# phymhan/pc-gan

Measured on AMD Instinct MI355X. Metric: images/sec (G+D step) 128x128 bs32 per GPU, higher is better.
Workload: dtype f32; 1 GPU; wsgan_emb UTKFace-shaped 128x128 bs32/GPU fp32: 9-block ResnetGenerator + 3-layer PatchGAN + ResNet-18 Elo encoder@224 + AlexNet IP@224, full optimize_parameters(); global_batch=32, parallelism=dp1

## Files before the change

### include/pcgan_hip.h

```cpp
#ifndef PCGAN_HIP_H
#define PCGAN_HIP_H

#include <stddef.h>
#include <stdint.h>

#ifdef __cplusplus
extern "C" {
#endif

typedef void* pcgan_stream_t;

const char* pcgan_last_error(void);
int pcgan_version(void);
int pcgan_device_info(int* cu_count, char* arch, int arch_len);

typedef struct {
    int N, C, H, W;
    int K, R, S;
    int stride, pad, pad_mode;
    int P, Q;
    int dtype;
} pcgan_conv_desc;

enum { PCGAN_ACT_NONE = 0, PCGAN_ACT_RELU = 1, PCGAN_ACT_LRELU = 2, PCGAN_ACT_TANH = 3, PCGAN_ACT_SIGMOID = 4 };
// ... 270 lines not shown
unsigned long long pcgan_pool_exchange_launches(void);

int pcgan_set_nonfinite_counter(unsigned int* dev_word);
int pcgan_set_option(const char* key, int value);
int pcgan_get_option(const char* key, int* value);
int pcgan_timer_enable(int capacity);
int pcgan_timer_read(int kind, float* ms, int cap);
#define PCGAN_IGEMM_LAUNCH_INFO 7
#define PCGAN_IGEMM_HGEMM_F16X2 1
#define PCGAN_IGEMM_HGEMM_BF16 2
#define PCGAN_IGEMM_IGEMM2_CG16 3
#define PCGAN_IGEMM_IGEMM2_CG4 4
#define PCGAN_IGEMM_GENERIC 5
#define PCGAN_IGEMM_SMALLM 6
int pcgan_igemm_last_launch(int* info, int n);
#define PCGAN_WGRAD_LAUNCH_INFO 9
#define PCGAN_WGRAD_TILE2 1
#define PCGAN_WGRAD_TILE 2
#define PCGAN_WGRAD_SMALLM 3
#define PCGAN_WGRAD_STRIP 4
int pcgan_wgrad_last_launch(int* info, int n);
#define PCGAN_HWGRAD_LAUNCH_INFO 12
int pcgan_hwgrad_last_launch(int* info, int n);

#ifdef __cplusplus
}
#endif
#endif
```

### pc-gan_amd/csrc/capi.hip

```cpp
#include "common.h"
#include <stdarg.h>
#include <atomic>
#include <mutex>
#include <vector>

namespace pcgan {
static thread_local char g_err[512] = "";
void set_error(const char* fmt, ...) {
    va_list ap;
    va_start(ap, fmt);
    vsnprintf(g_err, sizeof(g_err), fmt, ap);
    va_end(ap);
}
}

namespace pcgan {
namespace {
struct TimerKind {
    std::vector<hipEvent_t> start, stop;
    int used = 0;
};
std::mutex g_timer_mu;
std::atomic<int> g_timer_on{0};
TimerKind g_timer[TIMER_KINDS];
// ... 57 lines not shown
    }
    t.used = 0;
    return n;
}

namespace pcgan {
static std::atomic<unsigned*> g_nonfinite{nullptr};
unsigned* nonfinite_counter() { return g_nonfinite.load(std::memory_order_relaxed); }
}
extern "C" int pcgan_set_nonfinite_counter(unsigned int* dev_word) {
    pcgan::g_nonfinite.store(dev_word);
    return 0;
}

namespace pcgan {
static const char* const g_opt_names[OPT_COUNT] = {"bsplit_halo", "wgrad_gen", "wgrad_padcopy", "wgrad_cw", "hgemm_bf16", "wgd_look", "wgrad_direct", "hgemm_tile", "hgemm_ks", "wgrad_rowring", "wgrad_ks", "hwgrad_ks"};
static std::atomic<int> g_opt[OPT_COUNT] = {{1}, {1}, {0}, {0}, {1}, {3}, {0}, {0}, {0}, {1}, {0}, {0}};
int option(int id) { return (id >= 0 && id < OPT_COUNT) ? g_opt[id].load(std::memory_order_relaxed) : 0; }
static int option_index(const char* key) {
    for (int i = 0; key && i < OPT_COUNT; ++i)
        if (strcmp(key, g_opt_names[i]) == 0) return i;
    return -1;
}
}
extern "C" int pcgan_set_option(const char* key, int value) {
    using namespace pcgan;
    const int i = option_index(key);
    PCGAN_CHECK(i >= 0, "set_option: unknown option '%s' (bsplit_halo, wgrad_gen, wgrad_padcopy, wgrad_cw, hgemm_bf16, wgd_look, wgrad_direct, hgemm_tile, hgemm_ks, wgrad_rowring, wgrad_ks, hwgrad_ks)", key ? key : "(null)");
    PCGAN_CHECK(i != OPT_WGRAD_CW || value == 0 || value == 128 || value == 256, "set_option: wgrad_cw takes 0 (default), 128 or 256, got %d", value);
    PCGAN_CHECK(i != OPT_HGEMM_TILE || value == 0 || value == 128128 || value == 128064 || value == 64128 || value == 64064,
                "set_option: hgemm_tile takes 0 (heuristic) or BM * 1000 + BP with BM, BP in {64, 128}, got %d", value);
    PCGAN_CHECK(i != OPT_HGEMM_KS || (value >= 0 && value <= 8), "set_option: hgemm_ks takes 0 (heuristic) .. 8, got %d", value);
    PCGAN_CHECK(i != OPT_WGRAD_KS || (value >= 0 && value <= 512), "set_option: wgrad_ks takes 0 (heuristic) .. 512, got %d", value);
    PCGAN_CHECK(i != OPT_HWGRAD_KS || (value >= 0 && value <= 512), "set_option: hwgrad_ks takes 0 (heuristic) .. 512, got %d", value);
    g_opt[i].store(value);
    return 0;
}
extern "C" int pcgan_get_option(const char* key, int* value) {
    using namespace pcgan;
    const int i = option_index(key);
    PCGAN_CHECK(i >= 0 && value, "get_option: unknown option or null output");
    *value = g_opt[i].load();
    return 0;
// ... 20 lines not shown
```

### pc-gan_amd/csrc/common.h

```cpp
#pragma once
#include <hip/hip_runtime.h>
#include <stdint.h>
#include <stdio.h>
#include <string.h>
#include "../../include/pcgan_hip.h"

namespace pcgan {

void set_error(const char* fmt, ...);

#define PCGAN_CHECK(cond, ...)                \
    do {                                      \
        if (!(cond)) {                        \
            pcgan::set_error(__VA_ARGS__);    \
            return 1;                         \
        }                                     \
    } while (0)

#define PCGAN_LAUNCH_CHECK()                                                      \
    do {                                                                          \
        hipError_t e__ = hipGetLastError();                                       \
        if (e__ != hipSuccess) {                                                  \
            pcgan::set_error("%s:%d launch failed: %s", __FILE__, __LINE__,       \
                             hipGetErrorString(e__));                             \
// ... 1 lines not shown
        }                                                                         \
    } while (0)

enum { TIMER_RES_FWD = 0, TIMER_RES_DGRAD = 1, TIMER_RES_WGRAD = 2, TIMER_RES_WGRAD_MAIN = 3, TIMER_KINDS = 4 };
struct TimerScope {
    int kind, slot;
    hipStream_t st;
    TimerScope(int kind, hipStream_t st);
    ~TimerScope();
};

static inline int timer_kind_res(const pcgan_conv_desc* d, int kind) {
    return (d && d->K == 256 && d->C == 256 && d->R == 3 && d->S == 3 && d->stride == 1 && d->pad_mode == 1 && d->pad == 1) ? kind : -1;
}

enum { OPT_BSPLIT_HALO = 0, OPT_WGRAD_GEN = 1, OPT_WGRAD_PADCOPY = 2, OPT_WGRAD_CW = 3, OPT_HGEMM_BF16 = 4, OPT_WGD_LOOK = 5, OPT_WGRAD_DIRECT = 6, OPT_HGEMM_TILE = 7, OPT_HGEMM_KS = 8, OPT_WGRAD_ROWRING = 9, OPT_WGRAD_KS = 10, OPT_HWGRAD_KS = 11, OPT_COUNT = 12 };
int option(int id);

unsigned* nonfinite_counter();
int launch_wgd_reduce(const float* part, float* dw, const float* scales, int splits, int K, int C, int accumulate, hipStream_t st);
__device__ __forceinline__ bool is_nonfinite(float v) { return (__float_as_uint(v) & 0x7f800000u) == 0x7f800000u; }
__device__ __forceinline__ void report_nonfinite(unsigned* counter, bool bad) {
    if (counter != nullptr && __builtin_amdgcn_ballot_w64(bad) != 0ull && (threadIdx.x & 63) == 0) atomicAdd(counter, 1u);
}

int launch_weight_row_absmax(const float* w, int K, int C, int T, int by_c, float* out, hipStream_t st);

int launch_reflect_fold(const void* padded, void* dx, int NC, int H, int W, int pad, int dtype, hipStream_t st, const float* bias = nullptr,
                        int C = 1);

static inline int ilog2_exact(int v) {
// ... 176 lines not shown
```

### pc-gan_amd/csrc/hgemm.hip

```cpp
#include "igemm.h"

namespace pcgan {

typedef _Float16 f16x8 __attribute__((ext_vector_type(8)));
typedef _Float16 f16x4 __attribute__((ext_vector_type(4)));

typedef __bf16 bf16x8v __attribute__((ext_vector_type(8)));
typedef __bf16 bf16x4v __attribute__((ext_vector_type(4)));

template <int MODE, int BM, int BP, typename TA>
__global__ void __launch_bounds__(256) hgemm_kernel(IgemmArgs a) {
    static_assert(MODE == MODE_FWD_ZERO || MODE == MODE_FWD_REFLECT || MODE == MODE_BWD, "forward and plain data gradient");
    constexpr bool HALF = sizeof(TA) == 2;
    constexpr int NP = HALF ? 1 : 2;
    constexpr unsigned ES = sizeof(TA);
    constexpr int WM = (BM == 128 || (BM == 64 && BP == 64)) ? 2 : 1;
    constexpr int WP = 4 / WM;
    constexpr int WMT = BM / WM, WPT = BP / WP;
    constexpr int MI = WMT / 32, PJ = WPT / 32;
    constexpr int KPT = BP / 16;
    constexpr int ACH = BM * 4 / 256;
    constexpr int TROWS = NTAP_FWD + 1;
    constexpr int AH = BM + 8;
    __shared__ __attribute__((aligned(16))) f16x8 As[2][NP][2 * AH];
    __shared__ __attribute__((aligned(16))) f16x8 Bs[2][NP][2 * BP];
    __shared__ unsigned offT[TROWS][BP];
    __shared__ __attribute__((aligned(16))) float biasS[BM];
    __shared__ __attribute__((aligned(16))) float iswS[BM];

    const int nMt = (a.M + BM - 1) / BM;
    const int mt = blockIdx.x % nMt;
    int pt = blockIdx.x / nMt;
    int phase = 0;
    while (phase + 1 < a.nphase && pt >= a.tstart[phase + 1]) ++phase;
    pt -= a.tstart[phase];
    const PhaseArgs& P = a.ph[phase];
    const int tid = threadIdx.x;
    const int lane = tid & 63, lo = lane & 31, hi = lane >> 5;
    const int wave = __builtin_amdgcn_readfirstlane(tid >> 6);
    const int wm = wave / WP, wp = wave % WP;
    const int Ptot = P.Ptot, Kp = P.Kp;
    const int m0 = mt * BM, p0 = pt * BP;
    const int ph_nS = P.nS;
    const int T = P.nR * ph_nS;
    const int HgWg4 = a.Hg * a.Wg * (int)ES;
    const __amdgpu_buffer_rsrc_t rX = make_rsrc(a.X, a.x_bytes);
    const __amdgpu_buffer_rsrc_t rA = make_rsrc(P.A, (unsigned)a.M * (unsigned)Kp * 4u);

    float sx = 1.f;
    const int pl = tid % BP;
    {
        const int pg = p0 + pl;
        const bool pvalid = pg < Ptot;
        int gn = 0, py = 0, px = 0;
        if (pvalid) pix_coord(a, P, pg, gn, py, px);
        const unsigned vbase = (unsigned)gn * (unsigned)a.Cg * (unsigned)(a.Hg * a.Wg);
        for (int t = tid / BP; t <= T; t += 256 / BP) {
            const int ri = t / ph_nS, sj = t - ri * ph_nS;
            const int r = P.r0 + ri * a.tstep, sxx = P.s0 + sj * a.tstep;
            const bool live = pvalid && t < T;
            const unsigned y = axis_entry<MODE>(py, py + a.pad, true, r, a.Hg, a.sl, a.pad);
            const unsigned x = axis_entry<MODE>(px, px + a.pad, true, sxx, a.Wg, a.sl, a.pad);
            offT[t][pl] = (live && y != 0xffffffffu && x != 0xffffffffu) ? (vbase + y * (unsigned)a.Wg + x) * ES : OOB;
        }
    }
    const int ksub = __builtin_amdgcn_readfirstlane(tid / BP);
// ... 7 lines not shown

    int it_tap, it_c, it_k0, it_left = nst_here;
    {
        const int cc0 = st_begin / T;
        it_tap = st_begin - cc0 * T;
        it_c = cc0 * 16;
        it_k0 = st_begin * 16;
    }
    unsigned a_base[ACH];
#pragma unroll
    for (int j = 0; j < ACH; ++j) {
        const int q = tid + 256 * j;
        const int row = q >> 2, kc = (q & 3) * 4;
        a_base[j] = (m0 + row < a.M) ? (unsigned)((m0 + row) * Kp + kc) * 4u : OOB;
    }
    struct Stage {
        u32x4 av[ACH];
        unsigned bv[KPT];
    };
    auto load = [&](Stage& r) {
        const bool live = it_left > 0;
        const unsigned vo = offT[live ? it_tap : T][pl];
        const unsigned so = (unsigned)((it_c + ksub * KPT) * HgWg4);
#pragma unroll
        for (int j = 0; j < ACH; ++j) r.av[j] = __builtin_amdgcn_raw_buffer_load_b128(rA, live ? a_base[j] : OOB, (unsigned)it_k0 * 4u, 0);
#pragma unroll
        for (int i = 0; i < KPT; ++i) {
            if constexpr (HALF) r.bv[i] = (unsigned)__builtin_amdgcn_raw_buffer_load_b16(rX, vo, so + (unsigned)(i * HgWg4), 0);
            else r.bv[i] = __builtin_amdgcn_raw_buffer_load_b32(rX, vo, so + (unsigned)(i * HgWg4), 0);
        }
        --it_left;
        const int t1 = it_tap + 1;
        const bool wr = t1 == T;
        it_tap = wr ? 0 : t1;
        it_c += wr ? 16 : 0;
        it_k0 += 16;
    };
    auto stash = [&](const Stage& r, int buf) {
        if constexpr (HALF) {
#pragma unroll
            for (int j = 0; j < ACH; ++j) {
                const int q = tid + 256 * j;
                const int row = q >> 2, kc = (q & 3) * 4;
                bf16x4v h;
// ... 10 lines not shown
            return;
        }
#pragma unroll
        for (int j = 0; j < ACH; ++j) {
            const int q = tid + 256 * j;
            const int row = q >> 2, kc = (q & 3) * 4;
            typedef unsigned u32x2 __attribute__((ext_vector_type(2)));
            u32x2 h, l;
            h[0] = r.av[j][0]; h[1] = r.av[j][1];
            l[0] = r.av[j][2]; l[1] = r.av[j][3];
            _Float16* d0 = reinterpret_cast<_Float16*>(&As[buf][0][(kc >> 3) * AH + row]) + (kc & 4);
            _Float16* d1 = reinterpret_cast<_Float16*>(&As[buf][NP - 1][(kc >> 3) * AH + row]) + (kc & 4);
            *reinterpret_cast<u32x2*>(d0) = h;
            *reinterpret_cast<u32x2*>(d1) = l;
        }
        if constexpr (KPT == 8) {
            f16x8 h, l;
#pragma unroll
            for (int e = 0; e < 8; ++e) {
                _Float16 x, y;
                split2h(__uint_as_float(r.bv[e]) * sx, x, y);
                h[e] = x;
                l[e] = y;
            }
            Bs[buf][0][ksub * BP + pl] = h;
            Bs[buf][NP - 1][ksub * BP + pl] = l;
        } else {
            f16x4 h, l;
#pragma unroll
            for (int e = 0; e < 4; ++e) {
                _Float16 x, y;
// ... 4 lines not shown
            *reinterpret_cast<f16x4*>(reinterpret_cast<_Float16*>(&Bs[buf][0][(ksub >> 1) * BP + pl]) + (ksub & 1) * 4) = h;
            *reinterpret_cast<f16x4*>(reinterpret_cast<_Float16*>(&Bs[buf][NP - 1][(ksub >> 1) * BP + pl]) + (ksub & 1) * 4) = l;
        }
    };

    f32x16 acc[MI][PJ];
#pragma unroll
    for (int i = 0; i < MI; ++i)
#pragma unroll
        for (int j = 0; j < PJ; ++j)
#pragma unroll
            for (int r = 0; r < 16; ++r) acc[i][j][r] = 0.f;
    struct Operands {
        f16x8 A[NP][MI], B[NP][PJ];
    };
    auto fetch = [&](Operands& o, int buf) {
#pragma unroll
        for (int p = 0; p < NP; ++p) {
#pragma unroll
            for (int i = 0; i < MI; ++i) o.A[p][i] = As[buf][p][hi * AH + wm * WMT + i * 32 + lo];
#pragma unroll
            for (int j = 0; j < PJ; ++j) o.B[p][j] = Bs[buf][p][hi * BP + wp * WPT + j * 32 + lo];
        }
    };
    auto mma = [&](const Operands& o) {
        if constexpr (HALF) {
#pragma unroll
            for (int i = 0; i < MI; ++i)
#pragma unroll
                for (int j = 0; j < PJ; ++j)
                    acc[i][j] = __builtin_amdgcn_mfma_f32_32x32x16_bf16(__builtin_bit_cast(bf16x8v, o.A[0][i]), __builtin_bit_cast(bf16x8v, o.B[0][j]),
                                                                         acc[i][j], 0, 0, 0);
            return;
        }
        constexpr int PA[3] = {NP - 1, 0, 0}, PB[3] = {0, NP - 1, 0};
#pragma unroll
        for (int q = 0; q < 3; ++q)
#pragma unroll
            for (int i = 0; i < MI; ++i)
#pragma unroll
                for (int j = 0; j < PJ; ++j)
                    acc[i][j] = __builtin_amdgcn_mfma_f32_32x32x16_f16(o.A[PA[q]][i], o.B[PB[q]][j], acc[i][j], 0, 0, 0);
    };
    auto interleave = [&]() {
        constexpr int NM = (HALF ? 1 : 3) * MI * PJ, NRD = NP * (MI + PJ);
#pragma unroll
        for (int q = 0; q < NM; ++q) {
            __builtin_amdgcn_sched_group_barrier(0x008, 1, 0);
            __builtin_amdgcn_sched_group_barrier(0x100, (NRD + NM - 1) / NM, 0);
            __builtin_amdgcn_sched_group_barrier(0x002, 48 / NM + 1, 0);
            __builtin_amdgcn_sched_group_barrier(0x200, 1, 0);
            __builtin_amdgcn_sched_group_barrier(0x020, (ACH + KPT + NM - 1) / NM, 0);
        }
    };

    Stage rg[2];
    if (nst_here > 0) {
        load(rg[0]);
        load(rg[1]);
    }
    if constexpr (!HALF) {
        const float m = thread_max_of_partials(a.x_amax, a.x_namax, tid, 256);
        sx = pow2_scale(block_max(m, biasS));
        if (tid < BM) iswS[tid] = m0 + tid < a.M ? 1.f / pow2_scale(a.w_amax[m0 + tid]) : 1.f;
        __syncthreads();
    }
    if (tid < BM) biasS[tid] = (a.bias != nullptr && m0 + tid < a.M) ? a.bias[m0 + tid] : 0.f;
    if (nst_here == 0) __syncthreads();
    if (nst_here > 0) {
        Operands op[2];
        stash(rg[0], 0);
        __syncthreads();
        load(rg[0]);
        fetch(op[0], 0);
        stash(rg[1], 1);
        __syncthreads();
        load(rg[1]);
        const int nst2 = (nst_here + 1) & ~1;
        for (int s = 0; s < nst2; s += 2) {
#pragma unroll
            for (int t = 0; t < 2; ++t) {
                fetch(op[t ^ 1], t ^ 1);
                mma(op[t]);
                stash(rg[t], t);
                load(rg[t]);
// ... 41 lines not shown
#pragma unroll
            for (int r = 0; r < 16; ++r) {
                const int ml = wm * WMT + i * 32 + (r & 3) + 8 * (r >> 2) + 4 * hi;
                if (m0 + ml < a.M) st1(Yp + (size_t)(m0 + ml) * YhYw, act_apply((acc[i][j][r] * isx) * (HALF ? 1.f : iswS[ml]) + biasS[ml], a.act, a.slope));
            }
    }
}

template <int MODE>
static void launch_mode(const IgemmArgs& a, int bm, int bp, dim3 grid2, hipStream_t st) {
    if (bm == 128 && bp == 128) LAUNCH_TA(a.dtype, hgemm_kernel, grid2, a, MODE, 128, 128);
    else if (bm == 128) LAUNCH_TA(a.dtype, hgemm_kernel, grid2, a, MODE, 128, 64);
    else if (bp == 128) LAUNCH_TA(a.dtype, hgemm_kernel, grid2, a, MODE, 64, 128);
    else LAUNCH_TA(a.dtype, hgemm_kernel, grid2, a, MODE, 64, 64);
}
int launch_hgemm(int mode, const IgemmArgs& a, int bm, int bp, dim3 grid2, hipStream_t st) {
    switch (mode) {
        case MODE_FWD_ZERO: launch_mode<MODE_FWD_ZERO>(a, bm, bp, grid2, st); break;
        case MODE_FWD_REFLECT: launch_mode<MODE_FWD_REFLECT>(a, bm, bp, grid2, st); break;
        case MODE_BWD: launch_mode<MODE_BWD>(a, bm, bp, grid2, st); break;
        default: PCGAN_CHECK(false, "hgemm: no kernel for mode %d", mode);
    }
    PCGAN_LAUNCH_CHECK();
    return 0;
}

}

using namespace pcgan;

__global__ void __launch_bounds__(256) hgemm_presplit_kernel(float* __restrict__ A, int M, int Kp4, const float* __restrict__ rowmax) {
// ... 21 lines not shown
```

### pc-gan_amd/csrc/igemm.h

```cpp
#pragma once
#include "common.h"
#include <type_traits>

namespace pcgan {

typedef float f32x16 __attribute__((ext_vector_type(16)));

enum { MODE_FWD_ZERO = 0, MODE_FWD_REFLECT = 1, MODE_BWD = 2, MODE_BWD_REFLECT = 3 };

typedef unsigned int u32x4 __attribute__((ext_vector_type(4)));
static constexpr unsigned OOB = 0x80000000u;

__device__ __forceinline__ __amdgpu_buffer_rsrc_t make_rsrc(const void* p, unsigned bytes) {
    return __builtin_amdgcn_make_buffer_rsrc(const_cast<void*>(p), 0, (int)bytes, 0x00020000);
}
__device__ __forceinline__ float ld_b32(__amdgpu_buffer_rsrc_t r, unsigned voff, unsigned soff) {
    return __uint_as_float(__builtin_amdgcn_raw_buffer_load_b32(r, voff, soff, 0));
}
__device__ __forceinline__ float4 ld_b128(__amdgpu_buffer_rsrc_t r, unsigned voff) {
    const u32x4 v = __builtin_amdgcn_raw_buffer_load_b128(r, voff, 0, 0);
    return make_float4(__uint_as_float(v.x), __uint_as_float(v.y), __uint_as_float(v.z), __uint_as_float(v.w));
}

template <typename TA>
// ... 99 lines not shown
    int ostep, sl, pad, tstep;
    int act;
    float slope;
    unsigned x_bytes;
    int nphase;
    int rowfold;
    int chunked;
    int ksplit;
    float* Ypart;
    int tstart[17];
    PhaseArgs ph[16];
    const float* x_amax;
    const float* w_amax;
    int x_namax, hsplit;
    unsigned* ovf;
};

struct Geom {
    int Hg, Wg, sl, pad;
};

template <int MODE>
__device__ __forceinline__ bool tap_offset(const Geom& a, int py, int px, int r, int s, int& off) {
    if (MODE == MODE_BWD || MODE == MODE_BWD_REFLECT) {
        const int ty = py + a.pad - r, tx = px + a.pad - s;
        const int oy = ty >> a.sl, ox = tx >> a.sl;
        off = oy * a.Wg + ox;
        return (ty >= 0) & (tx >= 0) & (oy < a.Hg) & (ox < a.Wg);
    } else {
        int iy = (py << a.sl) - a.pad + r;
// ... 83 lines not shown
static inline int round4(int v) { return (v + 3) & ~3; }
static inline size_t esz(const pcgan_conv_desc* d) { return d->dtype == PCGAN_BF16 ? 2 : 4; }

#define LAUNCH_TA(dt, KERNEL, GRID, ARG, ...)                                                                   \
    do {                                                                                                        \
        if ((dt) == PCGAN_BF16) hipLaunchKernelGGL((KERNEL<__VA_ARGS__, bf16>), GRID, dim3(256), 0, st, ARG);    \
        else hipLaunchKernelGGL((KERNEL<__VA_ARGS__, float>), GRID, dim3(256), 0, st, ARG);                      \
    } while (0)

void record_launch(int form, int mode, int bm, int bp, int ks, int nphase);
int launch_splitk_reduce(int dtype, hipStream_t st, const float* part, void* y, const float* bias, int ks, size_t out_elems, int M,
                         int HW, int act, float slope);

int launch_igemm_f32(int mode, const IgemmArgs& a, int bm, int bp, dim3 grid, dim3 grid2, hipStream_t st);
int launch_hgemm(int mode, const IgemmArgs& a, int bm, int bp, dim3 grid2, hipStream_t st);
int launch_hgemm_presplit(float* A, int M, int Kp4, const float* rowmax, hipStream_t st);
int launch_smallm(int mode, IgemmArgs& a, int pmax, hipStream_t st, float* part_ws, size_t part_bytes);
int launch_transpose4(const float* A, float* At, int M, int Kp, hipStream_t st);
int launch_pack_strip(const float* A, float* Ws, int M, int Cg, int Cgp, int nR, int nS, hipStream_t st);
int wgrad_splits(const pcgan_conv_desc* d, int* chunks_per_split);
int launch_wgrad(const pcgan_conv_desc* d, const WgradArgs& a, int splits, float* dw, int accumulate, hipStream_t st);

}
```

### pc-gan_amd/csrc/igemm_conv.hip

```cpp
#include "igemm.h"
#include <stdlib.h>
#include <mutex>

namespace pcgan {

template <typename TA>
__global__ void splitk_reduce_kernel(const float* __restrict__ part, TA* __restrict__ y, const float* __restrict__ bias,
                                     int ks, size_t n, int M, int HW, int act, float slope) {
    const size_t n4 = (n & 3) ? 0 : (n >> 2);
    const size_t stride = (size_t)gridDim.x * blockDim.x;
    for (size_t i = blockIdx.x * (size_t)blockDim.x + threadIdx.x; i < n4; i += stride) {
        float4 acc = reinterpret_cast<const float4*>(part)[i];
        for (int s = 1; s < ks; ++s) {
            const float4 v = reinterpret_cast<const float4*>(part + (size_t)s * n)[i];
            acc.x += v.x; acc.y += v.y; acc.z += v.z; acc.w += v.w;
        }
        float o[4] = {acc.x, acc.y, acc.z, acc.w};
#pragma unroll
        for (int u = 0; u < 4; ++u) {
            const size_t e = i * 4 + u;
            if (bias) o[u] += bias[(e / HW) % M];
            o[u] = act_apply(o[u], act, slope);
        }
        st4(y + 4 * i, make_float4(o[0], o[1], o[2], o[3]));
// ... 211 lines not shown
    if (m >= 64 && tile_blocks(M, ptot_max, nphase, m, p) < 384) p = 64;
    if (m == 128 && tile_blocks(M, ptot_max, nphase, m, p) < 384) m = 64;
    *bm = m;
    *bp = p;
}

static std::mutex g_launch_mu;
static int g_launch[PCGAN_IGEMM_LAUNCH_INFO] = {0};
void record_launch(int form, int mode, int bm, int bp, int ks, int nphase) {
    std::lock_guard<std::mutex> lk(g_launch_mu);
    const int seq = g_launch[0] + 1;
    const int v[PCGAN_IGEMM_LAUNCH_INFO] = {seq, form, mode, bm, bp, ks, nphase};
    for (int i = 0; i < PCGAN_IGEMM_LAUNCH_INFO; ++i) g_launch[i] = v[i];
}

static int launch_igemm(int mode, IgemmArgs& a, hipStream_t st, float* part_ws = nullptr, size_t part_bytes = 0) {
    int pmax = 0;
    for (int i = 0; i < a.nphase; ++i) pmax = a.ph[i].Ptot > pmax ? a.ph[i].Ptot : pmax;
    if (pmax <= 0 || a.nphase <= 0) return 0;
    if (a.M <= 4) return launch_smallm(mode, a, pmax, st, part_ws, part_bytes);
    int bm, bp, ks;
    int nst_min = 1 << 30;
    for (int i = 0; i < a.nphase; ++i) nst_min = (a.ph[i].Kp + 15) / 16 < nst_min ? (a.ph[i].Kp + 15) / 16 : nst_min;
    const size_t out_elems = (size_t)a.N * a.M * a.Yh * a.Yw;
    choose_tile(a.M, pmax, a.nphase, nst_min, part_ws != nullptr, &bm, &bp, &ks);
    if (ks > 1 && (size_t)ks * out_elems * 4 > part_bytes) ks = 1;
    a.ksplit = ks;
    a.Ypart = part_ws;
    const dim3 grid((unsigned)(((a.M + bm - 1) / bm) * ((pmax + bp - 1) / bp)), (unsigned)a.nphase, (unsigned)ks);
    a.tstart[0] = 0;
// ... 3 lines not shown
    PCGAN_CHECK(cg16 || mode != MODE_BWD_REFLECT, "igemm: fused reflect data-gradient needs K %% 16 == 0");
    if (cg4) {
        PCGAN_CHECK(a.Cgp == 4, "igemm: 4-channel stages need a 3-/4-channel tensor");
        for (int i = 0; i < a.nphase; ++i)
            PCGAN_CHECK(a.ph[i].nR * a.ph[i].nS <= NTAP_CG4, "igemm: 4-channel stages: more than %d taps", NTAP_CG4);
    }
    if (cg16) {
        PCGAN_CHECK((a.Cg % 16) == 0, "igemm: chunked K order needs a multiple of 16 channels");
        for (int i = 0; i < a.nphase; ++i)
            PCGAN_CHECK(a.ph[i].nR * a.ph[i].nS <= (mode == MODE_BWD_REFLECT ? NTAP_MIR : NTAP_FWD) && (a.ph[i].Kp % 16) == 0,
                        "igemm: chunked K order: bad phase");
    }
    const bool half = a.dtype == PCGAN_BF16 && option(OPT_HGEMM_BF16) != 0;
    if ((half || (a.hsplit && a.dtype == PCGAN_F32)) && cg16 && mode != MODE_BWD_REFLECT && bm >= 64) {
        record_launch(half ? PCGAN_IGEMM_HGEMM_BF16 : PCGAN_IGEMM_HGEMM_F16X2, mode, bm, bp, ks, a.nphase);
        if (int e = launch_hgemm(mode, a, bm, bp, grid2, st)) return e;
    } else {
        record_launch(cg16 ? PCGAN_IGEMM_IGEMM2_CG16 : (cg4 ? PCGAN_IGEMM_IGEMM2_CG4 : PCGAN_IGEMM_GENERIC), mode, bm, bp, ks, a.nphase);
        if (int e = launch_igemm_f32(mode, a, bm, bp, grid, grid2, st)) return e;
    }
    if (ks > 1 && launch_splitk_reduce(a.dtype, st, part_ws, a.Y, a.bias, ks, out_elems, a.M, a.Yh * a.Yw, a.act, a.slope)) return 2;
    return 0;
}

}

using namespace pcgan;

static size_t fwd_part_bytes(const pcgan_conv_desc* d) {
    const int ptot = d->N * d->P * d->Q;
// ... 315 lines not shown
    if (fwd) return launch_hgemm_presplit(packed, M, RS * round4(d->C) / 4, w_rowmax, st);
    BwdPlan pl;
    bwd_plan(d, pl);
    for (int i = 0; i < pl.n; ++i)
        if (int e = launch_hgemm_presplit(packed + pl.ph[i].a_off, M, pl.ph[i].nR * pl.ph[i].nS * round4(d->K) / 4, w_rowmax, st)) return e;
    return 0;
}

extern "C" int pcgan_igemm_last_launch(int* info, int n) {
    PCGAN_CHECK(info != nullptr && n > 0, "igemm_last_launch: null output");
    std::lock_guard<std::mutex> lk(g_launch_mu);
    for (int i = 0; i < n; ++i) info[i] = i < PCGAN_IGEMM_LAUNCH_INFO ? g_launch[i] : 0;
    return 0;
}

extern "C" size_t pcgan_conv2d_packed_bytes(const pcgan_conv_desc* d, int pass) {
    if (!d) return 0;
    if (pass == PCGAN_PASS_FWD) return fwd_base_bytes(d);
    if (pass == PCGAN_PASS_BWD_DATA) return bwd_base_bytes(d);
    return 0;
}
extern "C" int pcgan_conv2d_pack_weights(const pcgan_conv_desc* d, int pass, const float* w, float* packed,
                                         pcgan_stream_t s) {
    if (check_desc(d)) return 1;
    PCGAN_CHECK(w && packed, "conv2d_pack_weights: null pointer");
    if (pass == PCGAN_PASS_FWD) return pack_fwd(d, w, packed, (hipStream_t)s);
    PCGAN_CHECK(pass == PCGAN_PASS_BWD_DATA, "conv2d_pack_weights: pass %d has no packed weights", pass);
    PCGAN_CHECK(d->pad_mode == 0 || d->stride == 1, "conv2d_bwd_data: reflection padding needs stride 1");
    BwdPlan pl;
    bwd_plan(d, pl);
// ... 26 lines not shown
```

### pc-gan_amd/hip/lib.py

```python
import ctypes
import os

_HERE = os.path.dirname(os.path.abspath(__file__))
LIB_PATH = os.environ.get('PCGAN_LIB') or os.path.join(os.path.dirname(_HERE), 'lib', 'libpcgan_hip.so')

ACT_NONE, ACT_RELU, ACT_LRELU, ACT_TANH, ACT_SIGMOID = 0, 1, 2, 3, 4
PASS_FWD, PASS_BWD_DATA, PASS_BWD_WEIGHT = 0, 1, 2
F32, BF16 = 0, 1
ADD_N_MAX = 8
POOL_PLAN_MAX = 64
GCAM_TYPES = {'raw': 0, 'pw': 1, 'cw_pos': 2, 'pw_cw': 3}
POOL_PASS = -1


def pool_store(s):
    return 2 * int(s)


def pool_swap(s):
    return 2 * int(s) + 1


def pool_exchange_launches():
    return int(load().pcgan_pool_exchange_launches())
# ... 97 lines not shown
    'pcgan_event_destroy': (_i, [_vp]),
    'pcgan_resblock_supported': (_i, [_rp]),
    'pcgan_resblock_wgrad_workspace_bytes': (_sz, [_rp]),
    'pcgan_resblock_fwd': (_i, [_rp, _vp, _vp, _i, _vp, _vp, _vp, _vp, _vp, _vp, _vp, _vp, _vp, _vp, _vp, _vp, _vp, _vp, _vp]),
    'pcgan_resblock_bwd': (_i, [_rp, _vp, _vp, _vp, _i, _vp, _vp, _vp, _vp, _vp, _vp, _vp, _vp, _vp, _vp, _vp, _vp, _vp, _vp, _vp, _vp,
                                _vp, _sz, _vp, _vp, _vp]),
    'pcgan_set_nonfinite_counter': (_i, [_vp]),
    'pcgan_set_option': (_i, [ctypes.c_char_p, _i]),
    'pcgan_get_option': (_i, [ctypes.c_char_p, _vp]),
    'pcgan_timer_enable': (_i, [_i]),
    'pcgan_timer_read': (_i, [_i, _vp, _i]),
    'pcgan_igemm_last_launch': (_i, [ctypes.POINTER(_i), _i]),
    'pcgan_wgrad_last_launch': (_i, [ctypes.POINTER(_i), _i]),
    'pcgan_hwgrad_last_launch': (_i, [ctypes.POINTER(_i), _i]),
    'pcgan_conv2d_hgemm_supported': (_i, [_dp, _i]),
    'pcgan_conv2d_hgemm_pack': (_i, [_dp, _i, _vp, _vp, _vp, _vp]),
    'pcgan_conv2d_fwd_packed_hsplit': (_i, [_dp, _vp, _vp, _i, _vp, _vp, _vp, _vp, _i, _f, _vp, _sz, _vp]),
    'pcgan_conv2d_bwd_data_packed_hsplit': (_i, [_dp, _vp, _vp, _i, _vp, _vp, _vp, _vp, _vp, _sz, _vp]),
    'pcgan_conv2d_thin_supported': (_i, [_dp, _i]),
    'pcgan_conv2d_thin_packed_bytes': (_sz, [_dp, _i]),
    'pcgan_conv2d_thin_workspace_bytes': (_sz, [_dp, _i]),
    'pcgan_conv2d_thin_pack': (_i, [_dp, _i, _vp, _vp, _vp]),
    'pcgan_conv2d_fwd_thin': (_i, [_dp, _vp, _vp, _i, _vp, _vp, _vp, _i, _f, _vp]),
    'pcgan_conv2d_bwd_data_thin': (_i, [_dp, _vp, _vp, _i, _vp, _vp, _vp, _sz, _vp]),
    'pcgan_conv2d_hsplit_wgrad_supported': (_i, [_dp]),
    'pcgan_conv2d_hsplit_wgrad_inline': (_i, [_dp]),
    'pcgan_conv2d_hsplit_wgrad_workspace_bytes': (_sz, [_dp]),
    'pcgan_conv2d_bwd_weight_hsplit': (_i, [_dp, _vp, _vp, _i, _vp, _vp, _i, _vp, _i, _vp, _sz, _vp]),
    'pcgan_restrunk_fwd': (_i, [_rp, _i, _vp, _vp, _i] + [_vp] * 8 + [_vp] * 6 + [_vp]),
    'pcgan_restrunk_bwd': (_i, [_rp, _i, _vp, _vp, _vp, _i] + [_vp] * 6 + [_vp] * 6 + [_vp] * 6 + [_vp, _sz, _vp, _vp, _vp]),
# ... 48 lines not shown
    bundled = os.path.join(os.path.dirname(torch.__file__), 'lib', 'libamdhip64.so')
    if os.path.exists(bundled):
        ctypes.CDLL(bundled, mode=ctypes.RTLD_GLOBAL)
    lib = ctypes.CDLL(LIB_PATH)
    for name, (res, args) in SIGNATURES.items():
        fn = getattr(lib, name)
        fn.restype = res
        fn.argtypes = args
    _lib = lib
    _options_from_environment(lib)
    return lib


_ENV_OPTIONS = (('PCGAN_BSPLIT_HALO', 'bsplit_halo', int), ('PCGAN_WGRAD_GEN', 'wgrad_gen', int), ('PCGAN_WGRAD_PADCOPY', 'wgrad_padcopy', int),
                ('PCGAN_WGRAD_CW', 'wgrad_cw', int), ('PCGAN_HGEMM', 'hgemm_bf16', int), ('PCGAN_WGRAD_DIRECT', 'wgrad_direct', int),
                ('PCGAN_WGD_LOOK', 'wgd_look', int), ('PCGAN_WGRAD_ROWRING', 'wgrad_rowring', int))


def _options_from_environment(lib):
    for env, key, conv in _ENV_OPTIONS:
        v = os.environ.get(env)
        if v not in (None, ''):
            set_option(key, conv(v), lib)


def set_option(key, value, lib=None):
    lib = lib or load()
    if lib.pcgan_set_option(key.encode(), int(value)) != 0:
        msg = lib.pcgan_last_error()
        raise RuntimeError('pcgan_hip set_option failed: %s' % (msg.decode() if msg else '?'))

# ... 13 lines not shown
```

Before: 1233 images/sec.

## Stage shared input row-span window in LDS for fp32 hgemm conv

Adds a span variant of the split-fp16 hgemm conv kernel. It loads the padded input rows covered by a pixel tile into LDS once per channel group, split into hi/lo halves, and serves every filter tap from that window. This replaces per-tap gathered global loads of the im2col B operand. The goal is to remove repeated global reads of overlapping input pixels across the R*S taps. In exchange it uses dynamic LDS, adds window-fill synchronisation and index math, and is gated by a heuristic that is on by default for zero-pad or data-grad modes when the reuse ratio is high enough.

```diff
diff --git a/include/pcgan_hip.h b/include/pcgan_hip.h
--- a/include/pcgan_hip.h
+++ b/include/pcgan_hip.h
@@ -308,6 +308,9 @@
 #define PCGAN_IGEMM_GENERIC 5
 #define PCGAN_IGEMM_SMALLM 6
 int pcgan_igemm_last_launch(int* info, int n);
+#define PCGAN_HGEMM_SPAN_INFO 5
+int pcgan_conv2d_hgemm_span_entries(const pcgan_conv_desc* d, int pass);
+int pcgan_hgemm_span_last_launch(int* info, int n);
 #define PCGAN_WGRAD_LAUNCH_INFO 9
 #define PCGAN_WGRAD_TILE2 1
 #define PCGAN_WGRAD_TILE 2
diff --git a/pc-gan_amd/csrc/capi.hip b/pc-gan_amd/csrc/capi.hip
--- a/pc-gan_amd/csrc/capi.hip
+++ b/pc-gan_amd/csrc/capi.hip
@@ -95,8 +95,8 @@
 }
 
 namespace pcgan {
-static const char* const g_opt_names[OPT_COUNT] = {"bsplit_halo", "wgrad_gen", "wgrad_padcopy", "wgrad_cw", "hgemm_bf16", "wgd_look", "wgrad_direct", "hgemm_tile", "hgemm_ks", "wgrad_rowring", "wgrad_ks", "hwgrad_ks"};
-static std::atomic<int> g_opt[OPT_COUNT] = {{1}, {1}, {0}, {0}, {1}, {3}, {0}, {0}, {0}, {1}, {0}, {0}};
+static const char* const g_opt_names[OPT_COUNT] = {"bsplit_halo", "wgrad_gen", "wgrad_padcopy", "wgrad_cw", "hgemm_bf16", "wgd_look", "wgrad_direct", "hgemm_tile", "hgemm_ks", "wgrad_rowring", "wgrad_ks", "hwgrad_ks", "hgemm_span"};
+static std::atomic<int> g_opt[OPT_COUNT] = {{1}, {1}, {0}, {0}, {1}, {3}, {0}, {0}, {0}, {1}, {0}, {0}, {1}};
 int option(int id) { return (id >= 0 && id < OPT_COUNT) ? g_opt[id].load(std::memory_order_relaxed) : 0; }
 static int option_index(const char* key) {
     for (int i = 0; key && i < OPT_COUNT; ++i)
@@ -107,7 +107,7 @@
 extern "C" int pcgan_set_option(const char* key, int value) {
     using namespace pcgan;
     const int i = option_index(key);
-    PCGAN_CHECK(i >= 0, "set_option: unknown option '%s' (bsplit_halo, wgrad_gen, wgrad_padcopy, wgrad_cw, hgemm_bf16, wgd_look, wgrad_direct, hgemm_tile, hgemm_ks, wgrad_rowring, wgrad_ks, hwgrad_ks)", key ? key : "(null)");
+    PCGAN_CHECK(i >= 0, "set_option: unknown option '%s' (bsplit_halo, wgrad_gen, wgrad_padcopy, wgrad_cw, hgemm_bf16, wgd_look, wgrad_direct, hgemm_tile, hgemm_ks, wgrad_rowring, wgrad_ks, hwgrad_ks, hgemm_span)", key ? key : "(null)");
     PCGAN_CHECK(i != OPT_WGRAD_CW || value == 0 || value == 128 || value == 256, "set_option: wgrad_cw takes 0 (default), 128 or 256, got %d", value);
     PCGAN_CHECK(i != OPT_HGEMM_TILE || value == 0 || value == 128128 || value == 128064 || value == 64128 || value == 64064,
                 "set_option: hgemm_tile takes 0 (heuristic) or BM * 1000 + BP with BM, BP in {64, 128}, got %d", value);
diff --git a/pc-gan_amd/csrc/common.h b/pc-gan_amd/csrc/common.h
--- a/pc-gan_amd/csrc/common.h
+++ b/pc-gan_amd/csrc/common.h
@@ -39,7 +39,7 @@
     return (d && d->K == 256 && d->C == 256 && d->R == 3 && d->S == 3 && d->stride == 1 && d->pad_mode == 1 && d->pad == 1) ? kind : -1;
 }
 
-enum { OPT_BSPLIT_HALO = 0, OPT_WGRAD_GEN = 1, OPT_WGRAD_PADCOPY = 2, OPT_WGRAD_CW = 3, OPT_HGEMM_BF16 = 4, OPT_WGD_LOOK = 5, OPT_WGRAD_DIRECT = 6, OPT_HGEMM_TILE = 7, OPT_HGEMM_KS = 8, OPT_WGRAD_ROWRING = 9, OPT_WGRAD_KS = 10, OPT_HWGRAD_KS = 11, OPT_COUNT = 12 };
+enum { OPT_BSPLIT_HALO = 0, OPT_WGRAD_GEN = 1, OPT_WGRAD_PADCOPY = 2, OPT_WGRAD_CW = 3, OPT_HGEMM_BF16 = 4, OPT_WGD_LOOK = 5, OPT_WGRAD_DIRECT = 6, OPT_HGEMM_TILE = 7, OPT_HGEMM_KS = 8, OPT_WGRAD_ROWRING = 9, OPT_WGRAD_KS = 10, OPT_HWGRAD_KS = 11, OPT_HGEMM_SPAN = 12, OPT_COUNT = 13 };
 int option(int id);
 
 unsigned* nonfinite_counter();
diff --git a/pc-gan_amd/csrc/hgemm.hip b/pc-gan_amd/csrc/hgemm.hip
--- a/pc-gan_amd/csrc/hgemm.hip
+++ b/pc-gan_amd/csrc/hgemm.hip
@@ -8,9 +8,10 @@
 typedef __bf16 bf16x8v __attribute__((ext_vector_type(8)));
 typedef __bf16 bf16x4v __attribute__((ext_vector_type(4)));
 
-template <int MODE, int BM, int BP, typename TA>
+template <int MODE, int BM, int BP, typename TA, bool SPAN = false>
 __global__ void __launch_bounds__(256) hgemm_kernel(IgemmArgs a) {
     static_assert(MODE == MODE_FWD_ZERO || MODE == MODE_FWD_REFLECT || MODE == MODE_BWD, "forward and plain data gradient");
+    static_assert(!SPAN || (sizeof(TA) == 4 && MODE != MODE_FWD_REFLECT), "span form: fp32 tensors, zero padding or data gradient");
     constexpr bool HALF = sizeof(TA) == 2;
     constexpr int NP = HALF ? 1 : 2;
     constexpr unsigned ES = sizeof(TA);
@@ -25,6 +26,7 @@
     __shared__ __attribute__((aligned(16))) f16x8 As[2][NP][2 * AH];
     __shared__ __attribute__((aligned(16))) f16x8 Bs[2][NP][2 * BP];
     __shared__ unsigned offT[TROWS][BP];
+    extern __shared__ __attribute__((aligned(16))) f16x8 Win[];
     __shared__ __attribute__((aligned(16))) float biasS[BM];
     __shared__ __attribute__((aligned(16))) float iswS[BM];
 
@@ -49,7 +51,34 @@
 
     float sx = 1.f;
     const int pl = tid % BP;
-    {
+    const int EW = a.span_entries + 1, pitch = a.span_pitch;
+    unsigned* const woffS = reinterpret_cast<unsigned*>(Win + 8 * EW);
+    int Et = 0, UPS = 1, eb[PJ];
+    if constexpr (SPAN) {
+        const int Hp = a.Yh + P.nR - 1;
+        int n, py, px;
+        pix_coord(a, P, p0, n, py, px);
+        const int row0 = n * Hp + py;
+        const int plast = (p0 + BP < Ptot ? p0 + BP : Ptot) - 1;
+        pix_coord(a, P, plast, n, py, px);
+        Et = (n * Hp + py + P.nR - row0) * pitch;
+        UPS = (2 * Et + 256 * T - 1) / (256 * T);
+#pragma unroll
+        for (int j = 0; j < PJ; ++j) {
+            const int pix = p0 + wp * WPT + j * 32 + lo;
+            pix_coord(a, P, pix < Ptot ? pix : Ptot - 1, n, py, px);
+            eb[j] = (n * Hp + py - row0) * pitch + px + (MODE == MODE_BWD ? (P.nR - 1) * pitch + ph_nS - 1 : 0);
+        }
+        const int oy = MODE == MODE_BWD ? P.nR - 1 - a.pad : a.pad, ox = MODE == MODE_BWD ? ph_nS - 1 - a.pad : a.pad;
+        for (int e = tid; e < Et; e += 256) {
+            const int row = e / pitch, gr = row0 + row;
+            const int gn = gr / Hp;
+            const int iy = gr - gn * Hp - oy, ix = e - row * pitch - ox;
+            const bool ok = gn < a.N && (unsigned)iy < (unsigned)a.Hg && (unsigned)ix < (unsigned)a.Wg;
+            woffS[e] = ok ? (((unsigned)gn * (unsigned)a.Cg * (unsigned)a.Hg + (unsigned)iy) * (unsigned)a.Wg + (unsigned)ix) * ES : OOB;
+        }
+        if (tid < 8) Win[tid * EW + EW - 1] = f16x8{0, 0, 0, 0, 0, 0, 0, 0};
+    } else {
         const int pg = p0 + pl;
         const bool pvalid = pg < Ptot;
         int gn = 0, py = 0, px = 0;
@@ -87,20 +116,63 @@
         const int row = q >> 2, kc = (q & 3) * 4;
         a_base[j] = (m0 + row < a.M) ? (unsigned)((m0 + row) * Kp + kc) * 4u : OOB;
     }
+    constexpr int NBV = SPAN ? 8 : KPT;
     struct Stage {
         u32x4 av[ACH];
-        unsigned bv[KPT];
-    };
+        unsigned bv[NBV];
+        int wc, wk;
+    };
+    const int c_last = st_end > st_begin ? (st_end - 1) / T : -1;
+    auto wave_has = [&](int i) { return wave * 64 + 256 * i < 2 * Et; };
+    auto win_load = [&](unsigned (&bv)[NBV], int c, int i) {
+        const int u = tid + 256 * i, kh = u >= Et ? 1 : 0;
+        const bool ok = u < 2 * Et && c <= c_last;
+        const unsigned vo = (ok ? woffS[u - kh * Et] : OOB) + (unsigned)(kh * 8 * HgWg4);
+        const unsigned so = (unsigned)(c * 16 * HgWg4);
+#pragma unroll
+        for (int e = 0; e < 8; ++e) bv[e] = __builtin_amdgcn_raw_buffer_load_b32(rX, vo, so + (unsigned)(e * HgWg4), 0);
+    };
+    auto win_put = [&](const unsigned (&bv)[NBV], int c, int i) {
+        const int u = tid + 256 * i, kh = u >= Et ? 1 : 0;
+        if (u >= 2 * Et) return;
+        f16x8 h, l;
+#pragma unroll
+        for (int e = 0; e < 8; ++e) {
+            _Float16 x, y;
+            split2h(__uint_as_float(bv[e]) * sx, x, y);
+            h[e] = x;
+            l[e] = y;
+        }
+        f16x8* const w = Win + ((c & 1) * 4 + kh) * EW + (u - kh * Et);
+        w[0] = h;
+        w[2 * EW] = l;
+    };
+    auto win_sync = [&](int c, int i) {
+        if (!wave_has(i)) return;
+        unsigned bv[NBV];
+        win_load(bv, c, i);
+        win_put(bv, c, i);
+    };
+    int wi_c = (st_begin - 1 + T) / T, wi_k = (st_begin - 1 + T) % T;
     auto load = [&](Stage& r) {
         const bool live = it_left > 0;
-        const unsigned vo = offT[live ? it_tap : T][pl];
-        const unsigned so = (unsigned)((it_c + ksub * KPT) * HgWg4);
 #pragma unroll
         for (int j = 0; j < ACH; ++j) r.av[j] = __builtin_amdgcn_raw_buffer_load_b128(rA, live ? a_base[j] : OOB, (unsigned)it_k0 * 4u, 0);
-#pragma unroll
-        for (int i = 0; i < KPT; ++i) {
-            if constexpr (HALF) r.bv[i] = (unsigned)__builtin_amdgcn_raw_buffer_load_b16(rX, vo, so + (unsigned)(i * HgWg4), 0);
-            else r.bv[i] = __builtin_amdgcn_raw_buffer_load_b32(rX, vo, so + (unsigned)(i * HgWg4), 0);
+        if constexpr (SPAN) {
+            r.wc = wi_c;
+            r.wk = wi_k;
+            if (wave_has(wi_k * UPS)) win_load(r.bv, wi_c, wi_k * UPS);
+            const bool ww = wi_k + 1 == T;
+            wi_k = ww ? 0 : wi_k + 1;
+            wi_c += ww ? 1 : 0;
+        } else {
+            const unsigned vo = offT[live ? it_tap : T][pl];
+            const unsigned so = (unsigned)((it_c + ksub * KPT) * HgWg4);
+#pragma unroll
+            for (int i = 0; i < KPT; ++i) {
+                if constexpr (HALF) r.bv[i] = (unsigned)__builtin_amdgcn_raw_buffer_load_b16(rX, vo, so + (unsigned)(i * HgWg4), 0);
+                else r.bv[i] = __builtin_amdgcn_raw_buffer_load_b32(rX, vo, so + (unsigned)(i * HgWg4), 0);
+            }
         }
         --it_left;
         const int t1 = it_tap + 1;
@@ -141,7 +213,10 @@
             *reinterpret_cast<u32x2*>(d0) = h;
             *reinterpret_cast<u32x2*>(d1) = l;
         }
-        if constexpr (KPT == 8) {
+        if constexpr (SPAN) {
+            if (wave_has(r.wk * UPS)) win_put(r.bv, r.wc, r.wk * UPS);
+            for (int j = 1; j < UPS; ++j) win_sync(r.wc, r.wk * UPS + j);
+        } else if constexpr (KPT == 8) {
             f16x8 h, l;
 #pragma unroll
             for (int e = 0; e < 8; ++e) {
@@ -176,13 +251,32 @@
     struct Operands {
         f16x8 A[NP][MI], B[NP][PJ];
     };
+    int f_r = (st_begin % T) / ph_nS, f_s = (st_begin % T) % ph_nS, f_buf = (st_begin / T) & 1, f_left = nst_here;
+    int f_toff = f_r * pitch + f_s;
     auto fetch = [&](Operands& o, int buf) {
 #pragma unroll
         for (int p = 0; p < NP; ++p) {
 #pragma unroll
             for (int i = 0; i < MI; ++i) o.A[p][i] = As[buf][p][hi * AH + wm * WMT + i * 32 + lo];
-#pragma unroll
-            for (int j = 0; j < PJ; ++j) o.B[p][j] = Bs[buf][p][hi * BP + wp * WPT + j * 32 + lo];
+            if constexpr (!SPAN) {
+#pragma unroll
+                for (int j = 0; j < PJ; ++j) o.B[p][j] = Bs[buf][p][hi * BP + wp * WPT + j * 32 + lo];
+            }
+        }
+        if constexpr (SPAN) {
+            const f16x8* const w = Win + (f_buf * 4 + hi) * EW;
+#pragma unroll
+            for (int j = 0; j < PJ; ++j) {
+                const int ent = f_left > 0 ? (MODE == MODE_BWD ? eb[j] - f_toff : eb[j] + f_toff) : EW - 1;
+#pragma unroll
+                for (int p = 0; p < NP; ++p) o.B[p][j] = w[p * 2 * EW + ent];
+            }
+            const bool ws = f_s + 1 == ph_nS, wr = ws && f_r + 1 == P.nR;
+            --f_left;
+            f_toff = wr ? 0 : f_toff + (ws ? pitch - ph_nS + 1 : 1);
+            f_s = ws ? 0 : f_s + 1;
+            f_r = wr ? 0 : f_r + (ws ? 1 : 0);
+            f_buf ^= wr ? 1 : 0;
         }
     };
     auto mma = [&](const Operands& o) {
@@ -212,7 +306,7 @@
             __builtin_amdgcn_sched_group_barrier(0x100, (NRD + NM - 1) / NM, 0);
             __builtin_amdgcn_sched_group_barrier(0x002, 48 / NM + 1, 0);
             __builtin_amdgcn_sched_group_barrier(0x200, 1, 0);
-            __builtin_amdgcn_sched_group_barrier(0x020, (ACH + KPT + NM - 1) / NM, 0);
+            __builtin_amdgcn_sched_group_barrier(0x020, (ACH + NBV + NM - 1) / NM, 0);
         }
     };
 
@@ -231,6 +325,22 @@
     if (nst_here == 0) __syncthreads();
     if (nst_here > 0) {
         Operands op[2];
+        if constexpr (SPAN) {
+            const int c0 = st_begin / T, nsl = st_begin - 1 + T - c0 * T;
+            for (int q0 = 0; q0 < nsl * UPS; q0 += 4) {
+                unsigned bv[4][NBV];
+#pragma unroll
+                for (int b = 0; b < 4; ++b) {
+                    const int q = q0 + b;
+                    if (q < nsl * UPS && wave_has(q % (T * UPS))) win_load(bv[b], c0 + q / (T * UPS), q % (T * UPS));
+                }
+#pragma unroll
+                for (int b = 0; b < 4; ++b) {
+                    const int q = q0 + b;
+                    if (q < nsl * UPS && wave_has(q % (T * UPS))) win_put(bv[b], c0 + q / (T * UPS), q % (T * UPS));
+                }
+            }
+        }
         stash(rg[0], 0);
         __syncthreads();
         load(rg[0]);
@@ -302,7 +412,24 @@
     else if (bp == 128) LAUNCH_TA(a.dtype, hgemm_kernel, grid2, a, MODE, 64, 128);
     else LAUNCH_TA(a.dtype, hgemm_kernel, grid2, a, MODE, 64, 64);
 }
+template <int MODE>
+static void launch_span(const IgemmArgs& a, int bm, int bp, dim3 grid2, size_t lds, hipStream_t st) {
+    if (bm == 128 && bp == 128) hipLaunchKernelGGL((hgemm_kernel<MODE, 128, 128, float, true>), grid2, dim3(256), lds, st, a);
+    else if (bm == 128) hipLaunchKernelGGL((hgemm_kernel<MODE, 128, 64, float, true>), grid2, dim3(256), lds, st, a);
+    else if (bp == 128) hipLaunchKernelGGL((hgemm_kernel<MODE, 64, 128, float, true>), grid2, dim3(256), lds, st, a);
+    else hipLaunchKernelGGL((hgemm_kernel<MODE, 64, 64, float, true>), grid2, dim3(256), lds, st, a);
+}
+size_t hgemm_span_lds_bytes(int entries) { return (size_t)(entries + 1) * 8 * sizeof(f16x8) + (size_t)entries * 4; }
+size_t hgemm_static_lds_bytes(int bm) { return (size_t)8 * (bm + 8) * sizeof(f16x8) + (size_t)bm * 8; }
+
 int launch_hgemm(int mode, const IgemmArgs& a, int bm, int bp, dim3 grid2, hipStream_t st) {
+    if (a.span_entries > 0) {
+        PCGAN_CHECK(a.dtype == PCGAN_F32 && (mode == MODE_FWD_ZERO || mode == MODE_BWD), "hgemm: no span form for mode %d", mode);
+        if (mode == MODE_BWD) launch_span<MODE_BWD>(a, bm, bp, grid2, hgemm_span_lds_bytes(a.span_entries), st);
+        else launch_span<MODE_FWD_ZERO>(a, bm, bp, grid2, hgemm_span_lds_bytes(a.span_entries), st);
+        PCGAN_LAUNCH_CHECK();
+        return 0;
+    }
     switch (mode) {
         case MODE_FWD_ZERO: launch_mode<MODE_FWD_ZERO>(a, bm, bp, grid2, st); break;
         case MODE_FWD_REFLECT: launch_mode<MODE_FWD_REFLECT>(a, bm, bp, grid2, st); break;
diff --git a/pc-gan_amd/csrc/igemm.h b/pc-gan_amd/csrc/igemm.h
--- a/pc-gan_amd/csrc/igemm.h
+++ b/pc-gan_amd/csrc/igemm.h
@@ -137,6 +137,7 @@
     const float* w_amax;
     int x_namax, hsplit;
     unsigned* ovf;
+    int span_entries, span_pitch;
 };
 
 struct Geom {
@@ -250,6 +251,8 @@
 
 int launch_igemm_f32(int mode, const IgemmArgs& a, int bm, int bp, dim3 grid, dim3 grid2, hipStream_t st);
 int launch_hgemm(int mode, const IgemmArgs& a, int bm, int bp, dim3 grid2, hipStream_t st);
+size_t hgemm_span_lds_bytes(int entries);
+size_t hgemm_static_lds_bytes(int bm);
 int launch_hgemm_presplit(float* A, int M, int Kp4, const float* rowmax, hipStream_t st);
 int launch_smallm(int mode, IgemmArgs& a, int pmax, hipStream_t st, float* part_ws, size_t part_bytes);
 int launch_transpose4(const float* A, float* At, int M, int Kp, hipStream_t st);
diff --git a/pc-gan_amd/csrc/igemm_conv.hip b/pc-gan_amd/csrc/igemm_conv.hip
--- a/pc-gan_amd/csrc/igemm_conv.hip
+++ b/pc-gan_amd/csrc/igemm_conv.hip
@@ -249,6 +249,40 @@
     for (int i = 0; i < PCGAN_IGEMM_LAUNCH_INFO; ++i) g_launch[i] = v[i];
 }
 
+struct SpanGeom {
+    int rows, pitch, entries;
+};
+static int span_rows(int N, int Yh, int Yw, int R, int bp) {
+    const int q = Yh * Yw, ptot = N * q, Hp = Yh + R - 1;
+    int g = q, b = bp;
+    while (b) { const int t = g % b; g = b; b = t; }
+    const int ntiles = (ptot + bp - 1) / bp, period = q / g;
+    int worst = 0;
+    for (int t = 0; t < ntiles && t < period; ++t) {
+        const int first = t * bp, last = (first + bp < ptot ? first + bp : ptot) - 1;
+        const int rows = (last / q) * Hp + (last % q) / Yw - (first / q) * Hp - (first % q) / Yw + R;
+        worst = rows > worst ? rows : worst;
+    }
+    return worst;
+}
+static SpanGeom span_geom(bool unit, int mode, int N, int Yh, int Yw, int R, int S, int bm, int bp) {
+    SpanGeom g = {0, 0, 0};
+    if (!unit || option(OPT_HGEMM_SPAN) == 0 || (mode != MODE_FWD_ZERO && mode != MODE_BWD)) return g;
+    g.rows = span_rows(N, Yh, Yw, R, bp);
+    g.pitch = Yw + S - 1;
+    const long entries = (long)g.rows * g.pitch;
+    if (entries > 4096 || hgemm_span_lds_bytes((int)entries) + hgemm_static_lds_bytes(bm) > 80 * 1024) return g;
+    if (option(OPT_HGEMM_SPAN) == 1 && (long)R * S * bp < 8 * entries) return g;
+    g.entries = (int)entries;
+    return g;
+}
+static int g_span[PCGAN_HGEMM_SPAN_INFO] = {0};
+static void record_span(const SpanGeom& g) {
+    std::lock_guard<std::mutex> lk(g_launch_mu);
+    const int v[PCGAN_HGEMM_SPAN_INFO] = {g_span[0] + 1, g.entries > 0, g.rows, g.pitch, g.entries};
+    for (int i = 0; i < PCGAN_HGEMM_SPAN_INFO; ++i) g_span[i] = v[i];
+}
+
 static int launch_igemm(int mode, IgemmArgs& a, hipStream_t st, float* part_ws = nullptr, size_t part_bytes = 0) {
     int pmax = 0;
     for (int i = 0; i < a.nphase; ++i) pmax = a.ph[i].Ptot > pmax ? a.ph[i].Ptot : pmax;
@@ -282,6 +316,11 @@
     const bool half = a.dtype == PCGAN_BF16 && option(OPT_HGEMM_BF16) != 0;
     if ((half || (a.hsplit && a.dtype == PCGAN_F32)) && cg16 && mode != MODE_BWD_REFLECT && bm >= 64) {
         record_launch(half ? PCGAN_IGEMM_HGEMM_BF16 : PCGAN_IGEMM_HGEMM_F16X2, mode, bm, bp, ks, a.nphase);
+        const SpanGeom sg = span_geom(!half && a.nphase == 1 && a.sl == 0 && a.ostep == 1 && a.tstep == 1, mode, a.N, a.Yh, a.Yw,
+                                      a.ph[0].nR, a.ph[0].nS, bm, bp);
+        a.span_entries = sg.entries;
+        a.span_pitch = sg.pitch;
+        record_span(sg);
         if (int e = launch_hgemm(mode, a, bm, bp, grid2, st)) return e;
     } else {
         record_launch(cg16 ? PCGAN_IGEMM_IGEMM2_CG16 : (cg4 ? PCGAN_IGEMM_IGEMM2_CG4 : PCGAN_IGEMM_GENERIC), mode, bm, bp, ks, a.nphase);
@@ -627,6 +666,21 @@
     return 0;
 }
 
+extern "C" int pcgan_hgemm_span_last_launch(int* info, int n) {
+    PCGAN_CHECK(info != nullptr && n > 0, "hgemm_span_last_launch: null output");
+    std::lock_guard<std::mutex> lk(g_launch_mu);
+    for (int i = 0; i < n; ++i) info[i] = i < PCGAN_HGEMM_SPAN_INFO ? g_span[i] : 0;
+    return 0;
+}
+extern "C" int pcgan_conv2d_hgemm_span_entries(const pcgan_conv_desc* d, int pass) {
+    if (!d || d->stride != 1 || d->pad_mode != 0 || !pcgan_conv2d_hgemm_supported(d, pass)) return 0;
+    const bool fwd = pass == PCGAN_PASS_FWD;
+    const int M = fwd ? d->K : d->C, Yh = fwd ? d->P : d->H, Yw = fwd ? d->Q : d->W;
+    int bm, bp, ks;
+    choose_tile(M, d->N * Yh * Yw, 1, d->R * d->S * round4(fwd ? d->C : d->K) / 16, (fwd ? fwd_part_bytes(d) : bwd_part_bytes(d)) != 0, &bm, &bp, &ks);
+    return span_geom(true, fwd ? MODE_FWD_ZERO : MODE_BWD, d->N, Yh, Yw, d->R, d->S, bm, bp).entries;
+}
+
 extern "C" size_t pcgan_conv2d_packed_bytes(const pcgan_conv_desc* d, int pass) {
     if (!d) return 0;
     if (pass == PCGAN_PASS_FWD) return fwd_base_bytes(d);
diff --git a/pc-gan_amd/hip/lib.py b/pc-gan_amd/hip/lib.py
--- a/pc-gan_amd/hip/lib.py
+++ b/pc-gan_amd/hip/lib.py
@@ -135,6 +135,8 @@
     'pcgan_wgrad_last_launch': (_i, [ctypes.POINTER(_i), _i]),
     'pcgan_hwgrad_last_launch': (_i, [ctypes.POINTER(_i), _i]),
     'pcgan_conv2d_hgemm_supported': (_i, [_dp, _i]),
+    'pcgan_conv2d_hgemm_span_entries': (_i, [_dp, _i]),
+    'pcgan_hgemm_span_last_launch': (_i, [ctypes.POINTER(_i), _i]),
     'pcgan_conv2d_hgemm_pack': (_i, [_dp, _i, _vp, _vp, _vp, _vp]),
     'pcgan_conv2d_fwd_packed_hsplit': (_i, [_dp, _vp, _vp, _i, _vp, _vp, _vp, _vp, _i, _f, _vp, _sz, _vp]),
     'pcgan_conv2d_bwd_data_packed_hsplit': (_i, [_dp, _vp, _vp, _i, _vp, _vp, _vp, _vp, _vp, _sz, _vp]),
@@ -213,7 +215,7 @@
 
 _ENV_OPTIONS = (('PCGAN_BSPLIT_HALO', 'bsplit_halo', int), ('PCGAN_WGRAD_GEN', 'wgrad_gen', int), ('PCGAN_WGRAD_PADCOPY', 'wgrad_padcopy', int),
                 ('PCGAN_WGRAD_CW', 'wgrad_cw', int), ('PCGAN_HGEMM', 'hgemm_bf16', int), ('PCGAN_WGRAD_DIRECT', 'wgrad_direct', int),
-                ('PCGAN_WGD_LOOK', 'wgd_look', int), ('PCGAN_WGRAD_ROWRING', 'wgrad_rowring', int))
+                ('PCGAN_WGD_LOOK', 'wgd_look', int), ('PCGAN_WGRAD_ROWRING', 'wgrad_rowring', int), ('PCGAN_HGEMM_SPAN', 'hgemm_span', int))
 
 
 def _options_from_environment(lib):
```

Result: no change. 1233 images/sec (-0.0%).
